# Stebalien/drand

Hardware: AMD Instinct MI355X
Metric: verified beacon rounds/sec, 10M-round chained BLS12-381 chain (higher is better)
Workload: dtype u32 (14x28-bit limb Fp, int32 VALU); 1 GPU; configs[1] shape at the metric's size: chained G2 chain, per-round pairing verify; rounds_total=10000000, rounds_per_gpu=10000000, seg_len=64, scheme=pedersen-bls-chained, mode=per-round, parallelism=shard1

## Files before the change

### __graft_entry__.py

```python
import json
import os
import subprocess
import sys

ROOT = os.path.dirname(os.path.abspath(__file__))
CSRC = os.path.join(ROOT, "drand_amd", "csrc")
LIB = os.path.join(ROOT, "drand_amd", "libdrand_gpu.so")
AB_LIB = os.path.join(ROOT, "drand_amd", "libdrand_gpu_ab.so")
INGEST = os.path.join(ROOT, "drand_amd", "libdrand_ingest.so")
HOSTSIM_SRC = os.path.join(ROOT, "tests", "hostsim", "hostsim.hip")
HOSTSIM = os.path.join(ROOT, "tests", "hostsim", "libdrand_hostsim.so")


def _run(cmd):
    print("+", " ".join(cmd), flush=True)
    subprocess.check_call(cmd, cwd=ROOT)


def build():
    os.environ.setdefault("PYTORCH_ROCM_ARCH", "gfx950")
    hip = ["hipcc", "--offload-arch=gfx950", "-O3", "-std=c++17", "-shared", "-fPIC"]
    ab_cmd = hip + ["-DDG_AB_KNOBS", "-o", AB_LIB, os.path.join(CSRC, "capi.hip")]
    print("+", " ".join(ab_cmd), "&", flush=True)
    ab = subprocess.Popen(ab_cmd, cwd=ROOT)
    try:
        _run(hip + ["-o", LIB, os.path.join(CSRC, "capi.hip")])
    finally:
        if ab.wait() != 0:
            raise subprocess.CalledProcessError(ab.returncode, ab_cmd)
    _run(["g++", "-O3", "-std=c++17", "-fPIC", "-shared", "-Wall", "-o", INGEST, os.path.join(CSRC, "ingest.cpp")])
    _run(["hipcc", "-O2", "-std=c++17", "--cuda-host-only", "-fPIC", "-shared", "-o", HOSTSIM, HOSTSIM_SRC])
    _run(["hipcc", "-O2", "-std=c++17", "--cuda-host-only", "-fPIC", "-shared", "-o",
          os.path.join(ROOT, "tests", "hostsim", "libdrand_reduce_lazy.so"),
          os.path.join(ROOT, "tests", "hostsim", "reduce_lazy.hip")])
    _run(["hipcc", "-O2", "-std=c++17", "--cuda-host-only", "-fPIC", "-shared", "-o",
          os.path.join(ROOT, "tests", "hostsim", "libdrand_miller6.so"),
          os.path.join(ROOT, "tests", "hostsim", "miller6.hip")])
    mk = os.path.join(ROOT, "oracle", "c", "Makefile")
    if os.path.exists(mk):
        _run(["make", "-C", os.path.join(ROOT, "oracle", "c"), "-j8"])
    sys.path.insert(0, ROOT)
    import drand_amd
    from drand_amd import _lib, ingest
    _lib.load()
    assert ingest.load() is not None


def smoke():
    sys.path.insert(0, ROOT)
    import torch
    assert torch.cuda.is_available(), "smoke() needs a GPU"
    from drand_amd.chain import Beacon, Verifier, hash_to_g2
    from drand_amd.scheme import get_scheme_by_id_with_default
    with open(os.path.join(ROOT, "tests", "golden", "chain_chained_s1.json")) as f:
        g = json.load(f)
    v = Verifier(get_scheme_by_id_with_default("pedersen-bls-chained"), device=0)
    beacons = [Beacon(bytes.fromhex(r["prev"]), r["round"], bytes.fromhex(r["sig"])) for r in g["rounds"][:8]]
    beacons += [Beacon(bytes.fromhex(c["prev"]), c["round"], bytes.fromhex(c["sig"])) for c in g["corrupted"]]
    expect = [0] * 8 + [c["reason"] for c in g["corrupted"]]
    got = v.verify_reasons(beacons, bytes.fromhex(g["pk"])).tolist()
    assert got == expect, (got, expect)
    with open(os.path.join(ROOT, "tests", "golden", "hash_to_g2.json")) as f:
        h = json.load(f)["cases"][:4]
    out = hash_to_g2([bytes.fromhex(c["msg"]) for c in h])
    assert [o.hex() for o in out] == [c["h"] for c in h]
    print("smoke ok:", len(beacons), "beacons verified on", torch.cuda.get_device_name(0))


if __name__ == "__main__":
    build()
```

### drand_amd/_lib.py

```python
import ctypes
import sys
import os
import threading

_HERE = os.path.dirname(os.path.abspath(__file__))
LIB_PATH = os.environ.get("DRAND_GPU_LIB") or os.path.join(_HERE, "libdrand_gpu.so")
AB_LIB_PATH = os.path.join(_HERE, "libdrand_gpu_ab.so")
AB_KNOBS = frozenset({"DGPU_DEC_OVERLAP", "DGPU_MSM_SEG", "DGPU_LANE_SLICES", "DGPU_KB_NORM", "DGPU_RLC_DESCENT_STEP",
                      "DGPU_RLC_LOCALIZE", "DGPU_G1_LINES", "DGPU_SUBGROUP", "DGPU_RECOVER", "DGPU_RECOVER_ROWS",
                      "DGPU_KB_INV_CHAIN", "DGPU_KB_TEST_FLAG", "DGPU_TEST_ALLOC_CAP", "DGPU_STAGE",
                      "DGPU_ENG_XW", "DGPU_TEST_STAGE_ONLY", "DGPU_LINES_WAVE", "DGPU_KB_PAIR", "DGPU_TEST_FORCE_EXC",
                      "DGPU_REDUCE_NORM", "DGPU_KEYED_RANGE", "DGPU_TEST_MILLER_MARK"})

DGPU_OK = 0
DGPU_EINVAL = -1
DGPU_EDEVICE = -2
DGPU_ENOMEM = -3
DGPU_EUNSUPPORTED = -4
DGPU_ENOKEY = -5

SCHEME_CHAINED = 0
SCHEME_UNCHAINED = 1
SCHEME_UNCHAINED_G1 = 2
SCHEME_G1_RFC9380 = 3

MODE_PER_ROUND = 0
MODE_RLC = 1

REASON_OK = 0
REASON_DECODE = 1
REASON_SUBGROUP = 2
REASON_PAIRING = 3
REASON_INFINITY = 4
REASON_KEY = 5

_c = ctypes
_P = _c.c_void_p
SYMBOLS = [
    ("dgpu_abi_version", _c.c_int, []),
    ("dgpu_last_error", _c.c_char_p, []),
    ("dgpu_open", _c.c_int, [_c.c_int, _c.POINTER(_P)]),
    ("dgpu_close", None, [_P]),
    ("dgpu_scheme_from_name", _c.c_int, [_c.c_char_p]),
    ("dgpu_set_pubkey", _c.c_int, [_P, _c.c_int, _P, _c.c_size_t]),
    ("dgpu_verify_batch", _c.c_int, [_P, _c.c_int, _c.c_size_t, _P, _P, _c.c_size_t, _P, _P, _c.c_size_t, _P,
                                     _c.c_int, _c.c_uint64, _P, _P]),
    ("dgpu_verify_batch_device", _c.c_int, [_P, _c.c_int, _c.c_size_t, _P, _P, _c.c_size_t, _P, _P, _c.c_size_t,
                                            _P, _c.c_int, _c.c_uint64, _P, _P, _P]),
    ("dgpu_set_profiling", _c.c_int, [_P, _c.c_int]),
    ("dgpu_staging_stats", _c.c_int, [_P, _c.POINTER(_c.c_double), _c.POINTER(_c.c_double), _c.POINTER(_c.c_uint64)]),
    ("dgpu_synchronize", _c.c_int, [_P]),
    ("dgpu_stage_times", _c.c_int, [_P, _c.POINTER(_c.c_float), _c.c_int, _c.POINTER(_c.c_char_p)]),
    ("dgpu_digest_batch", _c.c_int, [_P, _c.c_int, _c.c_size_t, _P, _P, _c.c_size_t, _P, _P]),
    ("dgpu_hash_to_g2", _c.c_int, [_P, _c.c_size_t, _P, _P]),
    ("dgpu_hash_to_g1", _c.c_int, [_P, _c.c_int, _c.c_size_t, _P, _P]),
    ("dgpu_derive_pubkey", _c.c_int, [_P, _c.c_int, _P, _P, _c.c_size_t]),
    ("dgpu_make_chain", _c.c_int, [_P, _c.c_int, _P, _c.c_size_t, _c.c_size_t, _P, _P, _P, _P]),
    ("dgpu_set_group", _c.c_int, [_P, _c.c_int, _c.c_int, _P]),
    ("dgpu_set_group_scheme", _c.c_int, [_P, _c.c_int, _c.c_int, _c.c_int, _P, _c.c_size_t]),
    ("dgpu_recover_batch_device", _c.c_int, [_P, _c.c_size_t, _P, _c.c_size_t, _P, _c.c_size_t, _P, _P, _P, _P, _P]),
    ("dgpu_make_partials", _c.c_int, [_P, _c.c_size_t, _P, _c.c_size_t, _P, _P, _P, _c.c_size_t, _P]),
    ("dgpu_make_partials_scheme", _c.c_int, [_P, _c.c_int, _c.c_size_t, _P, _c.c_size_t, _P, _P, _P, _c.c_size_t,
                                             _P]),
    ("dgpu_recover_batch", _c.c_int, [_P, _c.c_size_t, _P, _c.c_size_t, _P, _c.c_size_t, _P, _P, _P, _P]),
    ("dgpu_shard_range", None, [_c.c_size_t, _c.c_int, _c.c_int, _c.POINTER(_c.c_size_t), _c.POINTER(_c.c_size_t)]),
    ("dgpu_verify_beacons", _c.c_int, [_P, _c.c_int, _P, _c.c_size_t, _c.c_size_t, _P, _P, _c.c_size_t, _P, _P,
                                       _c.c_size_t, _P, _c.c_int, _c.c_uint64, _P, _P]),
    ("dgpu_verify_beacons_device", _c.c_int, [_P, _c.c_int, _P, _c.c_size_t, _c.c_size_t, _P, _P, _c.c_size_t, _P,
                                              _P, _c.c_size_t, _P, _c.c_int, _c.c_uint64, _P, _P, _P]),
    ("dgpu_decode_rows_device", _c.c_int, [_P, _c.c_size_t, _P, _c.c_size_t, _P, _P, _P, _P, _c.c_size_t, _P, _P,
                                           _c.c_size_t, _P, _P, _P]),
    ("dgpu_verify_rows", _c.c_int, [_P, _c.c_int, _P, _c.c_size_t, _c.c_size_t, _P, _P, _P, _c.c_size_t, _c.c_size_t,
                                    _c.c_int, _c.c_uint64, _P, _P, _P, _P]),
    ("dgpu_faulty_rounds_device", _c.c_int, [_P, _c.c_uint64, _c.c_size_t, _c.c_size_t, _P, _P, _P, _P, _P, _P,
                                             _c.c_size_t, _P, _c.c_size_t, _P, _P]),
    ("dgpu_check_rows", _c.c_int, [_P, _c.c_int, _P, _c.c_size_t, _c.c_size_t, _P, _P, _P, _P, _c.c_size_t,
                                   _c.c_size_t, _c.c_int, _c.c_uint64, _c.c_uint64, _c.c_size_t, _P, _P, _c.c_size_t,
                                   _P, _P, _c.c_size_t, _P, _P]),
    ("dgpu_verify_segment", _c.c_int, [_P, _c.c_int, _P, _c.c_size_t, _c.c_uint64, _c.c_size_t, _P, _c.c_size_t, _P,
                                       _P, _c.c_size_t, _c.c_int, _c.c_uint64, _P, _P, _P]),
    ("dgpu_verify_segment_device", _c.c_int, [_P, _c.c_int, _P, _c.c_size_t, _c.c_uint64, _c.c_size_t, _P,
                                              _c.c_size_t, _P, _P, _c.c_size_t, _c.c_int, _c.c_uint64, _P, _P, _P,
                                              _P]),
    ("dgpu_verify_segment_shard_device", _c.c_int, [_P, _c.c_int, _P, _c.c_size_t, _c.c_uint64, _c.c_size_t, _P,
                                                    _c.c_size_t, _P, _P, _P, _c.c_int, _c.c_uint64, _P, _P, _P, _P]),
    ("dgpu_rlc_root_segment_device", _c.c_int, [_P, _c.c_int, _P, _c.c_size_t, _c.c_uint64, _c.c_size_t, _P,
                                                _c.c_size_t, _P, _P, _c.c_size_t, _P, _P, _c.c_uint64, _P, _P]),
    ("dgpu_rlc_root_bytes", _c.c_int, [_c.c_int]),
    ("dgpu_rlc_root_device", _c.c_int, [_P, _c.c_int, _P, _c.c_size_t, _c.c_size_t, _P, _P, _c.c_size_t, _P, _P,
                                        _c.c_size_t, _P, _c.c_uint64, _P, _P]),
    ("dgpu_rlc_finish_device", _c.c_int, [_P, _c.c_size_t, _P, _P, _P, _P]),
    ("dgpu_verify_recovered", _c.c_int, [_P, _c.c_int, _P, _c.c_size_t, _c.c_size_t, _P, _c.c_size_t, _P, _P,
                                         _c.c_size_t, _P, _c.c_int, _c.c_uint64, _P, _P]),
    ("dgpu_hash_to_curve", _c.c_int, [_P, _c.c_int, _c.c_size_t, _P, _c.c_size_t, _P, _P]),
    ("dgpu_sign", _c.c_int, [_P, _c.c_int, _P, _c.c_size_t, _P, _c.c_size_t, _P, _P]),
# ... 148 lines not shown
```

### drand_amd/csrc/capi.hip

```cpp
#include <hip/hip_runtime.h>
#include <dlfcn.h>
#include <rccl/rccl.h>
#include <algorithm>
#include <atomic>
#include <chrono>
#include <condition_variable>
#include <deque>
#include <cstdarg>
#include <cstdio>
#include <cstdlib>
#include <cstring>
#include <mutex>
#include <random>
#include <string>
#include <thread>
#include <vector>

#include "../../include/drand_gpu.h"
#include "copy_pool.h"
#include "kernels.cuh"
#include "pairing_engine.cuh"
#include "miller6_kernels.cuh"
#include "lines_thread.cuh"
#include "kb_thread.cuh"
#include "recover.cuh"
#include "g1sig.cuh"
#include "rlc_msm.cuh"
#include "recover_g1.cuh"
#include "ingest_row.cuh"
#include "check_rows.cuh"
#include "keyed.cuh"
#include "scratch_layouts.h"
#include "record_arrays.h"

using namespace dgpu;

namespace {

thread_local std::string g_last_error;

int set_err(int code, const char* fmt, ...) __attribute__((format(printf, 2, 3)));
int set_err(int code, const char* fmt, ...) {
  char buf[512];
  va_list ap;
  va_start(ap, fmt);
  vsnprintf(buf, sizeof buf, fmt, ap);
  va_end(ap);
  g_last_error = buf;
  return code;
}

#define HIP_TRY(expr)                                                                             \
  do {                                                                                            \
    hipError_t _e = (expr);                                                                       \
    if (_e != hipSuccess) return set_err(DGPU_EDEVICE, "%s: %s", #expr, hipGetErrorString(_e)); \
  } while (0)
#define RC_TRY(expr)                  \
  do {                                \
    if (int _rc = (expr)) return _rc; \
  } while (0)

#ifdef DG_AB_KNOBS
size_t g_test_alloc_cap = 0;
#endif
struct DevBuf {
  void* p = nullptr;
  size_t cap = 0;
  DevBuf() = default;
  DevBuf(const DevBuf&) = delete;
  DevBuf& operator=(const DevBuf&) = delete;
  DevBuf(DevBuf&& o) noexcept : p(o.p), cap(o.cap) { o.p = nullptr, o.cap = 0; }
  DevBuf& operator=(DevBuf&& o) noexcept {
    if (this != &o) {
      release();
      p = o.p, cap = o.cap;
      o.p = nullptr, o.cap = 0;
    }
    return *this;
  }
  ~DevBuf() { release(); }
  int ensure(size_t bytes) {
    if (bytes <= cap) return DGPU_OK;
#ifdef DG_AB_KNOBS
    if (g_test_alloc_cap && bytes > g_test_alloc_cap)
      return set_err(DGPU_ENOMEM, "hipMalloc(%zu): test cap %zu", bytes, g_test_alloc_cap);
#endif
    if (p) {
      (void)hipDeviceSynchronize();
      (void)hipFree(p);
    }
    p = nullptr;
    cap = 0;
    hipError_t e = hipMalloc(&p, bytes ? bytes : 1);
    if (e != hipSuccess) return set_err(DGPU_ENOMEM, "hipMalloc(%zu): %s", bytes, hipGetErrorString(e));
    cap = bytes;
    return DGPU_OK;
  }
  void release() {
    if (p) (void)hipFree(p);
    p = nullptr;
    cap = 0;
  }
  template <class T>
  T* as() const { return static_cast<T*>(p); }
  uint32_t* u32() const { return as<uint32_t>(); }
// ... 39 lines not shown
  z = (z ^ (z >> 30)) * 0xBF58476D1CE4E5B9ull;
  z = (z ^ (z >> 27)) * 0x94D049BB133111EBull;
  return z ^ (z >> 31);
}

inline bool sig_on_g1(int scheme) { return scheme == DGPU_SCHEME_UNCHAINED_G1 || scheme == DGPU_SCHEME_G1_RFC9380; }
inline bool scheme_known(int scheme) { return scheme >= DGPU_SCHEME_CHAINED && scheme <= DGPU_SCHEME_G1_RFC9380; }

constexpr size_t ENG_CHUNK = 1048576;
constexpr size_t ENG_CHUNK_MIN = 16384;
constexpr size_t LANE_MIN = 262144;
constexpr int KEY_SLOTS = 8;
constexpr size_t STAGE_SLOT_BYTES = 16u << 20;
constexpr int STAGE_COPY_THREADS = 8;

struct lane_scratch {
  DevBuf h_pts, sig_pts, h_z, h_pre, h_tmp;
  DevBuf lines, f, n1, kb;
};

struct key_entry {
  bool used = false;
  bool g2key = false;
  uint8_t bytes[96] = {};
  g1_key pk{};
  DevBuf consts, table;
  uint64_t stamp = 0;
};

template <class F>
auto with_src(const msg_src_host& m, F&& f) {
  if (m.linked == SRC_HALO) {
    msg_src_halo h{};
    static_cast<msg_src&>(h) = m;
    h.first_round = m.first_round;
    h.g0 = m.g0;
    h.halo = m.halo;
    h.halo_len = m.halo_len;
    return f(static_cast<const msg_src_halo&>(h));
  }
  return m.linked ? f(static_cast<const msg_src_linked&>(m)) : f(static_cast<const msg_src&>(m));
}
#define SRC_KERNEL(K, src) K<std::decay_t<decltype(src)>>

template <class F>
auto with_group(bool g1, F&& f) {
  return g1 ? f(G1Ops{}) : f(G2Ops{});
}
#define GROUP_OF(gr) std::decay_t<decltype(gr)>

}

struct dgpu_ctx {
  int device = -1;
  hipStream_t stream = nullptr;
  hipStream_t stream2 = nullptr;
  hipEvent_t lane_ev[2] = {nullptr, nullptr};
  hipEvent_t cof_ev[2] = {nullptr, nullptr};
  hipEvent_t done = nullptr;
  std::mutex mu;
  key_entry keys[KEY_SLOTS];
  key_entry* cur = nullptr;
  uint64_t clock = 0;
  DevBuf eng_consts;
  lane_scratch lane[2];
  DevBuf status;
  DevBuf rlc_tree, rlc_idx, rlc_fail, rlc_h, rlc_s, rlc_st, rlc_root;
  DevBuf rlc_conf, rlc_fsum;
  DevBuf msm_aos, msm_flags, msm_counts, msm_list, msm_buckets, msm_runs, msm_root, msm_part;
  bool fe_gs = false;
  size_t fe_gs_max = 16384;
  size_t kb_inv_chain = 16;
  size_t kb_test_flag = 0;
  int lanes = 2;
  size_t lane_slices = 2;
  size_t eng_chunk = ENG_CHUNK;
  size_t chunk_retries = 0;
  bool kb_thread = true;
  bool kb_norm_chain = true;
  bool rlc_localize = true;
  int rlc_descent_step = 3;
  bool lines_thread = true;
  bool miller6 = true;
  size_t thr_min = 65536;
  size_t rlc_min = 131072;
  bool fused_fixed = true;
  bool decode_subgroup = false;
  int grp_t = 0, grp_n = 0;
  int grp_scheme = DGPU_SCHEME_CHAINED;
  bool grp_g1 = false;
  key_entry grp_key;
  DevBuf grp_stage, rec_slots;
  DevBuf grp_commits, grp_table, rec_msgs, rec_parts, rec_plen, rec_hidx, rec_pk, rec_idx, rec_lam, rec_out, rec_ok,
      rec_pts, rec_vpk, rec_sel, rec_part, rec_st;
  DevBuf grp_wtab, rec_cls, rec_x_list, rec_x_msgs, rec_x_parts, rec_x_plen, rec_x_out, rec_x_ok, rec_x_st;
  DevBuf rec_tab, rec_tabz, rec_tabpre;
  DevBuf rec_tab_rows;
  bool recover_exact = false;
  size_t cof_engine_max = 16384;
  DevBuf cof_tmp;
  bool dec_overlap = true;
  bool msm_seg = true;
  int n_cu = 256;
  bool recover_rows = true;
  void* ring[2] = {nullptr, nullptr};
  hipEvent_t ring_ev[2] = {nullptr, nullptr};
  bool ring_busy[2] = {false, false};
  int ring_next = 0;
  hipStream_t stream_copy = nullptr;
  float last_stage_ms = 0.f;
  double last_stage_host_ms = 0.0;
  bool test_stage_only = false;
  size_t last_stage_bytes = 0;
  bool test_miller_mark = false;
  bool kb_pair = false;
  bool reduce_norm = false;
  bool lines_wave = false;
  int eng_xw = 0;
  bool stage_pageable = false;
  DevBuf in_rounds, in_sigs, in_sig_len, in_prev, in_prev_len, in_msgs, in_msg_len, out_bits, out_reason, out_rand, misc;
  DevBuf in_rows, in_row_ok;
  DevBuf in_keys;
  DevBuf chk, chk_out;
  DevBuf in_halo, in_halo_len;
  DevBuf in_key_idx, ky_tab, ky_keys, ky_rlc, ky_exact;
  size_t keyed_range = 0;
  void* ky_host = nullptr;
  size_t ky_host_cap = 0;
  hipEvent_t ky_ev = nullptr;
  bool ky_ev_used = false;
  bool profile = false;
  std::vector<hipEvent_t> ev;
  std::vector<const char*> stage_name;
  int n_ev = 0;
  bool ev_overflow = false;
  bool rlc_pending = false;
  verify_args rlc_args{};
  uint8_t rlc_pk[96] = {};
  size_t rlc_pk_len = 0;
};

namespace {

struct stream_order {
  dgpu_ctx* c;
  hipStream_t s;
  stream_order(dgpu_ctx* c_, hipStream_t s_) : c(c_), s(s_) { (void)hipStreamWaitEvent(s, c->done, 0); }
  ~stream_order() { (void)hipEventRecord(c->done, s); }
};

template <int N>
struct stream_scratch {
  hipStream_t s;
  DevBuf b[N];
  explicit stream_scratch(hipStream_t s_) : s(s_) {}
  ~stream_scratch() { (void)hipStreamSynchronize(s); }
};

struct side_join {
  hipStream_t side, main;
  hipEvent_t ev;
  bool armed;
  side_join(hipStream_t side_, hipStream_t main_, hipEvent_t ev_) : side(side_), main(main_), ev(ev_), armed(side_ != nullptr) {}
  void release() { armed = false; }
  ~side_join() {
    if (armed && hipEventRecord(ev, side) == hipSuccess) (void)hipStreamWaitEvent(main, ev, 0);
  }
};

hipStream_t caller_stream(void* stream) { return (hipStream_t)stream; }

constexpr int STAGE_EVENTS_MAX = 4096;
void mark(dgpu_ctx* c, hipStream_t s, const char* name = nullptr) {
  if (!c->profile) return;
  if (c->n_ev >= STAGE_EVENTS_MAX) {
    c->ev_overflow = true;
    return;
  }
  if ((size_t)c->n_ev == c->ev.size()) {
    hipEvent_t e = nullptr;
    if (hipEventCreate(&e) != hipSuccess) return;
    c->ev.push_back(e);
    c->stage_name.push_back(nullptr);
  }
  (void)hipEventRecord(c->ev[c->n_ev], s);
  c->stage_name[c->n_ev] = name;
  c->n_ev++;
}

void call_reset(dgpu_ctx* c) {
  c->n_ev = 0;
  c->ev_overflow = false;
  c->rlc_pending = false;
}

int upload_eng_consts(DevBuf* dst, const g1_key* key, bool unit_points = false) {
  eng_const_block cb;
// ... 59 lines not shown
  memcpy(gw + 42, gen.y.c1.l, 56);
  hipStream_t s = c->stream;
  hipError_t err = hipMemcpyAsync(d_in, pk, 96, hipMemcpyHostToDevice, s);
  if (err == hipSuccess) err = hipMemcpyAsync(d_g2, gw, sizeof gw, hipMemcpyHostToDevice, s);
  if (err != hipSuccess) return set_err(DGPU_EDEVICE, "set_pubkey: %s", hipGetErrorString(err));
  RC_TRY(launch(k_decode_g2_pk, dim3(1), dim3(64), s, d_in, d_pk, d_rc));
  int drc = -1;
  err = hipMemcpyAsync(&drc, d_rc, sizeof drc, hipMemcpyDeviceToHost, s);
  if (err == hipSuccess) err = hipStreamSynchronize(s);
  if (err != hipSuccess) return set_err(DGPU_EDEVICE, "set_pubkey: %s", hipGetErrorString(err));
  if (drc != DEC_OK) return set_err(DGPU_EINVAL, "public key rejected (decode code %d)", drc);
  RC_TRY(launch(k_eng_lines, dim3(1), dim3(ENG_BLOCK), s, 1, 0, 1, d_pk, 1, nullptr, d_g2, nullptr, unit.u32(),
                e->table.u32(), nullptr, nullptr));
  err = hipStreamSynchronize(s);
  if (err != hipSuccess) return set_err(DGPU_EDEVICE, "set_pubkey lines: %s", hipGetErrorString(err));
  return DGPU_OK;
}

int get_key_locked(dgpu_ctx* c, int scheme, const uint8_t* pk, size_t len, key_entry** out) {
  if (!pk) return set_err(DGPU_EINVAL, "null public key");
  if (!scheme_known(scheme)) return set_err(DGPU_EINVAL, "bad scheme %d", scheme);
  const bool g2key = sig_on_g1(scheme);
  const size_t want = g2key ? 96 : 48;
  if (len != want)
    return set_err(DGPU_EINVAL, "public key must be %zu bytes (compressed %s), got %zu", want, g2key ? "G2" : "G1", len);
  key_entry* victim = nullptr;
  for (key_entry& e : c->keys) {
    if (e.used && e.g2key == g2key && !memcmp(e.bytes, pk, want)) {
      e.stamp = ++c->clock;
      *out = &e;
      return DGPU_OK;
    }
    if (!victim || (!e.used && victim->used) || (e.used == victim->used && e.stamp < victim->stamp)) victim = &e;
  }
  HIP_TRY(hipEventSynchronize(c->done));
  if (c->cur == victim) c->cur = nullptr;
  victim->used = false;
  int rc = g2key ? decode_g2_key_locked(c, victim, pk) : decode_g1_key_locked(c, victim, pk);
  if (rc) return rc;
  victim->used = true;
  victim->g2key = g2key;
  memcpy(victim->bytes, pk, want);
  victim->stamp = ++c->clock;
  *out = victim;
  return DGPU_OK;
}

int eng_fe_kb_locked(dgpu_ctx* c, const uint32_t* consts, size_t cnt, size_t capb, size_t r0, uint32_t* f,
                     const uint32_t* n1inv, const eng_kb_layout& kb, uint8_t* st, hipStream_t s) {
  if (capb % ENG_ROUNDS_PER_BLOCK || cnt > capb) return set_err(DGPU_EINVAL, "karabina FE: bad chunk capacity");
  uint32_t *const xbuf = kb.xbuf, *const pbuf = kb.pbuf, *const pre = kb.pre, *const ebuf = kb.ebuf, *const fb = kb.fb;
  uint8_t* const flags = kb.flags;
  const unsigned blocks = grid_for(cnt, ENG_ROUNDS_PER_BLOCK);
  const size_t inv_threads = std::max<size_t>(1, (cnt + c->kb_inv_chain - 1) / c->kb_inv_chain);
  constexpr int nseg = (int)(sizeof(ENG_PROG_FEK_OFF) / sizeof(ENG_PROG_FEK_OFF[0])) - 1;
  static_assert(nseg == 6, "segment 0 + one per exponentiation by |x|");
  for (int seg = 0; seg < nseg; ++seg) {
    if (seg > 0) {
      mark(c, s, "eng_fe_chain");
      const bool kb_thread = c->kb_thread && cnt >= c->thr_min;
      const bool norm_pre = kb_thread && c->kb_norm_chain;
      if (norm_pre && c->kb_pair)
        RC_TRY(launch_n(k_kb_chain_pair<true>, 2 * cnt, 256, s, cnt, xbuf, ebuf));
#ifdef DG_AB_KNOBS
      else if (kb_thread && c->reduce_norm)
        RC_TRY(launch_n(norm_pre ? k_kb_chain_thr<true, false> : k_kb_chain_thr<false, false>, cnt, 256, s, cnt, xbuf,
                        norm_pre ? ebuf : nullptr));
#endif
      else if (kb_thread)
        RC_TRY(launch_n(norm_pre ? k_kb_chain_thr<true> : k_kb_chain_thr<false>, cnt, 256, s, cnt, xbuf,
                        norm_pre ? ebuf : nullptr));
      else
        RC_TRY(launch(k_eng_kb_chain, dim3(grid_for(cnt, 8)), dim3(64), s, cnt, xbuf));
      mark(c, s, "eng_fe_kbinv");
      RC_TRY(launch_n(norm_pre ? k_eng_kb_norm<true> : k_eng_kb_norm<false>, cnt, 256, s, cnt, r0, xbuf, pbuf, ebuf, flags,
                      st, c->kb_test_flag));
      RC_TRY(launch_n(k_eng_inv, inv_threads, 256, s, cnt, r0, pbuf, pre, st));
      RC_TRY(launch_n(k_eng_kb_dec, (size_t)ENG_KB_NSNAP * cnt, 256, s, cnt, xbuf, pbuf, ebuf, flags));
    }
    mark(c, s, "eng_fe");
    const int so = ENG_PROG_FEK_OFF[seg], sl = ENG_PROG_FEK_OFF[seg + 1] - ENG_PROG_FEK_OFF[seg];
    const bool first = seg == 0, last = seg == nseg - 1;
#ifdef DG_AB_KNOBS
    if (c->eng_xw & 2)
      RC_TRY(launch(first || last ? k_eng_fe_seg_xw<ENG_SLOTS_FE> : k_eng_fe_seg_xw<ENG_FEK_MID_SLOTS>,
                    dim3(grid_for(cnt, ENG_XW_ITEMS)), dim3(ENG_XW_BLOCK), s, so, sl, first, last, cnt, r0, consts, f, n1inv,
                    xbuf, flags, fb, st));
    else
#endif
      RC_TRY(launch(k_eng_fe_seg, dim3(blocks), dim3(ENG_BLOCK), s, so, sl, first, last, cnt, r0, consts, f, n1inv, xbuf,
                    flags, fb, st));
  }
  return launch(k_eng_fe_fb, dim3(ENG_FB_GRID), dim3(ENG_BLOCK), s, cnt, r0, consts, f, n1inv, st, flags, fb);
}

struct pairing_job {
  const uint32_t* consts = nullptr;
  size_t n = 0;
  const uint32_t* h = nullptr;
  const uint32_t* sg = nullptr;
  uint8_t* st = nullptr;
  size_t h_stride = 0;
  const uint32_t* h_idx = nullptr;
  const uint32_t* pk_items = nullptr;
  const uint32_t* fixed_table = nullptr;
  lane_scratch* lane = nullptr;
  bool sig_subgroup = false;
  const uint32_t* g1form_keys = nullptr;
};

int eng_pairing_locked(dgpu_ctx* c, const pairing_job& job, hipStream_t s) {
  const uint32_t* const consts = job.consts;
  const size_t n = job.n;
  const uint32_t *const h = job.h, *const sg = job.sg;
  uint8_t* const st = job.st;
  const size_t h_stride = job.h_stride ? job.h_stride : n;
  const uint32_t *const h_idx = job.h_idx, *const pk_items = job.pk_items, *const fixed_table = job.fixed_table;
  lane_scratch& L = job.lane ? *job.lane : c->lane[0];
  const bool sig_subgroup = job.sig_subgroup;
  const uint32_t* const g1form_keys = job.g1form_keys;
  const bool need_lines = !(fixed_table && c->fused_fixed);
  const bool fe_gs = c->fe_gs || n <= c->fe_gs_max;
  int rc;
  size_t cap = 0, cap_blk = 0;
  eng_kb_layout kb{};
  bool retried = false;
  for (;;) {
    const size_t nchunks = (n + c->eng_chunk - 1) / c->eng_chunk;
    cap = (n + nchunks - 1) / nchunks;
    cap = std::min(n, (cap + ENG_ROUNDS_PER_BLOCK - 1) / ENG_ROUNDS_PER_BLOCK * ENG_ROUNDS_PER_BLOCK);
    cap_blk = eng_blocks(cap);
    rc = fe_gs ? DGPU_OK : carve(L.kb, &kb, cap_blk);
    if (!rc && need_lines) rc = L.lines.ensure(eng_blk_words(cap_blk, ENG_LINE_STEPS) * 4);
    if (!rc) rc = L.f.ensure(eng_blk_words(cap_blk, ENG_F_PLANES) * 4);
    if (!rc) rc = L.n1.ensure(eng_n1_words(cap) * 4);
    if (rc != DGPU_ENOMEM || c->eng_chunk <= ENG_CHUNK_MIN || cap <= ENG_CHUNK_MIN) break;
    HIP_TRY(hipStreamSynchronize(s));
    HIP_TRY(hipStreamSynchronize(c->stream));
    HIP_TRY(hipStreamSynchronize(c->stream2));
    for (DevBuf* b : {&L.kb, &L.lines, &L.f, &L.n1}) b->release();
    c->eng_chunk = std::max(ENG_CHUNK_MIN, c->eng_chunk / 2);
    ++c->chunk_retries;
    retried = true;
  }
  if (rc) return rc;
  if (retried) g_last_error.clear();
  uint32_t* lines = need_lines ? L.lines.u32() : nullptr;
  uint32_t* f = L.f.u32();
  uint32_t* n1 = L.n1.u32();
  uint32_t* pre = need_lines ? lines : nullptr;
  if (!pre) {
    if ((rc = c->lane[0].lines.ensure(eng_n1_words(cap) * 4))) return rc;
    pre = c->lane[0].lines.u32();
  }
  uint8_t* const sub_st = sig_subgroup ? st : nullptr;
  for (size_t r0 = 0; r0 < n; r0 += cap) {
    const size_t cnt = std::min(cap, n - r0);
    const dim3 blocks(grid_for(cnt, ENG_ROUNDS_PER_BLOCK)), eng(ENG_BLOCK);
    if (!need_lines) {
      mark(c, s, "eng_miller");
      RC_TRY(launch(k_eng_miller_fixed, blocks, eng, s, n, r0, cnt, consts, h, sg, fixed_table, f, n1));
    } else {
      const bool thr = c->lines_thread && cnt >= c->thr_min;
      if (g1form_keys) {
        mark(c, s, "eng_lines");
        RC_TRY(launch_n(k_lines_thr_g1, 2 * cnt, 256, s, n, r0, cnt, h, h_stride, h_idx, sg, g1form_keys, lines));
      } else if (fixed_table) {
        mark(c, s, "eng_lines_fixed");
        RC_TRY(launch(k_eng_lines_fixed, dim3(blocks.x, ENG_LINE_STEPS), eng, s, n, r0, cnt, h, sg, fixed_table, lines));
      } else if (thr && !pk_items && c->lines_wave) {
        mark(c, s, "eng_lines");
        RC_TRY(launch_n(k_lines_thr<true>, 2 * ((cnt + 63) / 64 * 64), 256, s, n, r0, cnt, h, h_stride, h_idx, sg, pk_items,
                        consts, lines, sub_st));
      } else if (thr) {
// ... 1085 lines not shown
  hipStream_t s = c->stream;
  stream_order ord(c, s);
  if (a.n && (rc = verify_status_host_locked(c, key, a, s))) return rc;
  if (a.n) mark(c, s);
  if ((rc = check_lists_locked(c, first, count, a.n, a.m.rows->d_keys, faulty_cap, left_cap, out, s))) return rc;
  if (reason && a.n) {
    HIP_TRY(hipMemcpyAsync(reason, c->status.p, a.n, hipMemcpyDeviceToHost, s));
    HIP_TRY(hipStreamSynchronize(s));
  }
  return DGPU_OK;
}

void check_lists_store(const check_lists& L, uint64_t* faulty_pos, uint64_t* faulty_val, size_t faulty_cap,
                       uint64_t* n_faulty, uint64_t* left_rows, size_t left_cap, uint64_t* n_left) {
  const size_t nf = std::min(L.pos.size(), faulty_cap), nl = std::min(L.left.size(), left_cap);
  if (nf) memcpy(faulty_pos, L.pos.data(), nf * 8), memcpy(faulty_val, L.val.data(), nf * 8);
  if (nl) memcpy(left_rows, L.left.data(), nl * 8);
  *n_faulty = L.n_faulty;
  *n_left = L.n_left;
}

size_t size_engine_chunk(int lanes) {
  size_t free_b = 0, total_b = 0;
  if (hipMemGetInfo(&free_b, &total_b) != hipSuccess) return ENG_CHUNK;
  const size_t fit = free_b / 2 / ((size_t)std::max(lanes, 1) * eng_bytes_per_round());
  return std::max(ENG_CHUNK_MIN, std::min(ENG_CHUNK, fit));
}

}

extern "C" {

int dgpu_abi_version(void) { return DGPU_ABI_VERSION; }
const char* dgpu_last_error(void) { return g_last_error.c_str(); }

int dgpu_scheme_from_name(const char* name) {
  if (!name) return set_err(DGPU_EINVAL, "null scheme name");
  if (name[0] == 0 || !strcmp(name, "pedersen-bls-chained")) return DGPU_SCHEME_CHAINED;
  if (!strcmp(name, "pedersen-bls-unchained")) return DGPU_SCHEME_UNCHAINED;
  if (!strcmp(name, "bls-unchained-on-g1")) return DGPU_SCHEME_UNCHAINED_G1;
  if (!strcmp(name, "bls-unchained-g1-rfc9380")) return DGPU_SCHEME_G1_RFC9380;
  return set_err(DGPU_EINVAL, "scheme [%s] is not valid", name);
}

void dgpu_shard_range(size_t n, int ndev, int k, size_t* lo, size_t* hi) {
  if (ndev < 1) ndev = 1;
  size_t per = (n + (size_t)ndev - 1) / (size_t)ndev;
  per = (per + 7) & ~(size_t)7;
  size_t a = std::min(n, (size_t)k * per), b = std::min(n, a + per);
  if (k < 0) a = b = 0;
  if (lo) *lo = a;
  if (hi) *hi = b;
}

int dgpu_open(int device, dgpu_ctx** out) {
  if (!out) return set_err(DGPU_EINVAL, "null out");
  *out = nullptr;
  int count = 0;
  hipError_t e = hipGetDeviceCount(&count);
  if (e != hipSuccess || count == 0) return set_err(DGPU_EDEVICE, "no HIP device available (%s)", hipGetErrorString(e));
  if (device < 0 || device >= count) return set_err(DGPU_EINVAL, "device %d out of range (%d devices)", device, count);
  hipDeviceProp_t prop;
  HIP_TRY(hipGetDeviceProperties(&prop, device));
  if (strncmp(prop.gcnArchName, "gfx950", 6) != 0)
    return set_err(DGPU_EDEVICE, "device %d is %s; this library is built for gfx950 only", device, prop.gcnArchName);
  HIP_TRY(hipSetDevice(device));
  dgpu_ctx* c = new dgpu_ctx();
  c->device = device;
  c->n_cu = prop.multiProcessorCount > 0 ? prop.multiProcessorCount : 256;
  const char* fgv = getenv("DGPU_FE_GS_MAX");
  if (fgv && atol(fgv) >= 0) c->fe_gs_max = (size_t)atol(fgv);
  const char* cev = getenv("DGPU_COF_ENGINE_MAX");
  if (cev && atol(cev) >= 0) c->cof_engine_max = (size_t)atol(cev);
  const char* lv = getenv("DGPU_LANES");
  if (lv && !strcmp(lv, "1")) c->lanes = 1;
  const char* ec = getenv("DGPU_ENG_CHUNK");
  c->eng_chunk = (ec && atol(ec) >= 4096) ? (size_t)atol(ec) : size_engine_chunk(c->lanes);
  const char* kcv = getenv("DGPU_KB_CHAIN");
  if (kcv && !strcmp(kcv, "lanes")) c->kb_thread = false;
  const char* lnv = getenv("DGPU_LINES");
  if (lnv && !strcmp(lnv, "engine")) c->lines_thread = false;
  const char* mlv = getenv("DGPU_MILLER");
  if (mlv && !strcmp(mlv, "lanes12")) c->miller6 = false;
  const char* tmv = getenv("DGPU_THR_MIN");
  if (tmv && atol(tmv) >= 0) c->thr_min = (size_t)atol(tmv);
  const char* rmv = getenv("DGPU_RLC_MIN");
  if (rmv && atol(rmv) >= 0) c->rlc_min = (size_t)atol(rmv);
  const char* fev = getenv("DGPU_FE");
  if (fev && !strcmp(fev, "gs")) c->fe_gs = true;
#ifdef DG_AB_KNOBS
  const char* dov = getenv("DGPU_DEC_OVERLAP");
  if (dov && !strcmp(dov, "0")) c->dec_overlap = false;
  const char* msv = getenv("DGPU_MSM_SEG");
  if (msv && !strcmp(msv, "0")) c->msm_seg = false;
  const char* lsv = getenv("DGPU_LANE_SLICES");
  if (lsv && atol(lsv) >= 2 && atol(lsv) <= 64) c->lane_slices = (size_t)atol(lsv);
  const char* knv = getenv("DGPU_KB_NORM");
  if (knv) c->kb_norm_chain = strcmp(knv, "planes") != 0;
  const char* rds = getenv("DGPU_RLC_DESCENT_STEP");
  if (rds && atoi(rds) >= 1 && atoi(rds) <= 8) c->rlc_descent_step = atoi(rds);
  const char* rlv = getenv("DGPU_RLC_LOCALIZE");
  if (rlv && !strcmp(rlv, "0")) c->rlc_localize = false;
  const char* gl = getenv("DGPU_G1_LINES");
  if (gl && !strcmp(gl, "buffer")) c->fused_fixed = false;
  const char* sgv = getenv("DGPU_SUBGROUP");
  if (sgv && !strcmp(sgv, "decode")) c->decode_subgroup = true;
  const char* rcv = getenv("DGPU_RECOVER");
  if (rcv && !strcmp(rcv, "exact")) c->recover_exact = true;
  const char* rrv = getenv("DGPU_RECOVER_ROWS");
  if (rrv && !strcmp(rrv, "0")) c->recover_rows = false;
  const char* kic = getenv("DGPU_KB_INV_CHAIN");
  if (kic && atol(kic) >= 1) c->kb_inv_chain = (size_t)atol(kic);
  const char* ktf = getenv("DGPU_KB_TEST_FLAG");
  if (ktf && atol(ktf) >= 1) c->kb_test_flag = (size_t)atol(ktf);
  const char* mmv = getenv("DGPU_TEST_MILLER_MARK");
  if (mmv) c->test_miller_mark = !strcmp(mmv, "1");
  const char* kpv = getenv("DGPU_KB_PAIR");
  if (kpv) c->kb_pair = !strcmp(kpv, "1");
  const char* rnv = getenv("DGPU_REDUCE_NORM");
  if (rnv) c->reduce_norm = !strcmp(rnv, "1");
  const char* lwv = getenv("DGPU_LINES_WAVE");
  if (lwv) c->lines_wave = !strcmp(lwv, "1");
  const char* xwv = getenv("DGPU_ENG_XW");
  if (xwv) c->eng_xw = atoi(xwv) & 3;
  const char* stv = getenv("DGPU_STAGE");
  if (stv && !strcmp(stv, "pageable")) c->stage_pageable = true;
  const char* krv = getenv("DGPU_KEYED_RANGE");
  if (krv && atol(krv) >= 1) c->keyed_range = (size_t)atol(krv);
  const char* tso = getenv("DGPU_TEST_STAGE_ONLY");
  if (tso && !strcmp(tso, "1")) c->test_stage_only = true;
  const char* tac = getenv("DGPU_TEST_ALLOC_CAP");
  g_test_alloc_cap = tac && atol(tac) >= 0 ? (size_t)atol(tac) : 0;
  {
    const char* fev2 = getenv("DGPU_TEST_FORCE_EXC");
    const int force = fev2 && !strcmp(fev2, "1") ? 1 : 0;
    const hipError_t fe = hipMemcpyToSymbol(HIP_SYMBOL(g_dg_force_exc), &force, sizeof(force));
    if (fe != hipSuccess) {
      delete c;
      return set_err(DGPU_EDEVICE, "DGPU_TEST_FORCE_EXC: %s", hipGetErrorString(fe));
    }
  }
#endif
  e = hipStreamCreateWithFlags(&c->stream, hipStreamNonBlocking);
  if (e == hipSuccess) e = hipStreamCreateWithFlags(&c->stream2, hipStreamNonBlocking);
  if (e == hipSuccess) e = hipEventCreateWithFlags(&c->lane_ev[0], hipEventDisableTiming);
  if (e == hipSuccess) e = hipEventCreateWithFlags(&c->lane_ev[1], hipEventDisableTiming);
  if (e == hipSuccess) e = hipEventCreateWithFlags(&c->cof_ev[0], hipEventDisableTiming);
  if (e == hipSuccess) e = hipEventCreateWithFlags(&c->cof_ev[1], hipEventDisableTiming);
  if (e == hipSuccess) e = hipEventCreateWithFlags(&c->done, hipEventDisableTiming);
  if (e != hipSuccess) {
    dgpu_close(c);
    return set_err(DGPU_EDEVICE, "hipStreamCreate: %s", hipGetErrorString(e));
  }
  if (upload_eng_consts(&c->eng_consts, nullptr) != DGPU_OK) {
    std::string msg = g_last_error;
    dgpu_close(c);
    return set_err(DGPU_EDEVICE, "%s", msg.c_str());
  }
  g_last_error.clear();
  *out = c;
  return DGPU_OK;
}

void dgpu_close(dgpu_ctx* c) {
  if (!c) return;
  (void)hipSetDevice(c->device);
  if (c->stream) (void)hipStreamSynchronize(c->stream);
  if (c->stream2) (void)hipStreamSynchronize(c->stream2);
  if (c->done) (void)hipEventSynchronize(c->done);
  for (hipEvent_t e : c->ev) (void)hipEventDestroy(e);
  for (hipEvent_t e : c->lane_ev)
    if (e) (void)hipEventDestroy(e);
  for (hipEvent_t e : c->cof_ev)
    if (e) (void)hipEventDestroy(e);
  if (c->done) (void)hipEventDestroy(c->done);
  if (c->ky_ev) (void)hipEventDestroy(c->ky_ev);
  if (c->ky_host) (void)hipHostFree(c->ky_host);
  if (c->stream_copy) {
    (void)hipStreamSynchronize(c->stream_copy);
    (void)hipStreamDestroy(c->stream_copy);
  }
  for (int k = 0; k < 2; ++k) {
    if (c->ring_ev[k]) (void)hipEventDestroy(c->ring_ev[k]);
    if (c->ring[k]) (void)hipHostFree(c->ring[k]);
  }
  if (c->stream2) (void)hipStreamDestroy(c->stream2);
  if (c->stream) (void)hipStreamDestroy(c->stream);
  delete c;
}

int dgpu_set_pubkey(dgpu_ctx* c, int scheme, const uint8_t* pk, size_t len) {
  if (!c || !pk) return set_err(DGPU_EINVAL, "null argument");
  std::lock_guard<std::mutex> lk(c->mu);
  HIP_TRY(hipSetDevice(c->device));
  key_entry* k = nullptr;
  int rc = get_key_locked(c, scheme, pk, len, &k);
  if (rc) return rc;
  c->cur = k;
  return DGPU_OK;
// ... 624 lines not shown
```

Before: 2.609 million rounds/s.

## Add six-lane final-exponentiation segment kernel reusing miller6 Fp12 layout

Adds a new kernel for the hard-part final-exponentiation segments (after segment 0). Each item is spread across six lanes that share Fp12 coefficients through LDS, reusing the miller6 multiply and square helpers. When the batch is at least the threshold size, this path replaces the 12-lane k_eng_fe_seg kernel. The goal is better lane utilisation and fewer registers per lane, at the cost of more LDS traffic and hand-written Frobenius and conjugation transforms that must match the old program exactly.

Result: faster. 2.652 million rounds/s, median of 6 (+1.6%).

```diff
diff --git a/__graft_entry__.py b/__graft_entry__.py
--- a/__graft_entry__.py
+++ b/__graft_entry__.py
@@ -36,6 +36,9 @@
     _run(["hipcc", "-O2", "-std=c++17", "--cuda-host-only", "-fPIC", "-shared", "-o",
           os.path.join(ROOT, "tests", "hostsim", "libdrand_miller6.so"),
           os.path.join(ROOT, "tests", "hostsim", "miller6.hip")])
+    _run(["hipcc", "-O2", "-std=c++17", "--cuda-host-only", "-fPIC", "-shared", "-o",
+          os.path.join(ROOT, "tests", "hostsim", "libdrand_feseg6.so"),
+          os.path.join(ROOT, "tests", "hostsim", "feseg6.hip")])
     mk = os.path.join(ROOT, "oracle", "c", "Makefile")
     if os.path.exists(mk):
         _run(["make", "-C", os.path.join(ROOT, "oracle", "c"), "-j8"])
diff --git a/drand_amd/_lib.py b/drand_amd/_lib.py
--- a/drand_amd/_lib.py
+++ b/drand_amd/_lib.py
@@ -10,7 +10,8 @@
                       "DGPU_RLC_LOCALIZE", "DGPU_G1_LINES", "DGPU_SUBGROUP", "DGPU_RECOVER", "DGPU_RECOVER_ROWS",
                       "DGPU_KB_INV_CHAIN", "DGPU_KB_TEST_FLAG", "DGPU_TEST_ALLOC_CAP", "DGPU_STAGE",
                       "DGPU_ENG_XW", "DGPU_TEST_STAGE_ONLY", "DGPU_LINES_WAVE", "DGPU_KB_PAIR", "DGPU_TEST_FORCE_EXC",
-                      "DGPU_REDUCE_NORM", "DGPU_KEYED_RANGE", "DGPU_TEST_MILLER_MARK"})
+                      "DGPU_REDUCE_NORM", "DGPU_KEYED_RANGE", "DGPU_TEST_MILLER_MARK",
+                      "DGPU_TEST_FE_MARK"})
 
 DGPU_OK = 0
 DGPU_EINVAL = -1
diff --git a/drand_amd/csrc/capi.hip b/drand_amd/csrc/capi.hip
--- a/drand_amd/csrc/capi.hip
+++ b/drand_amd/csrc/capi.hip
@@ -21,6 +21,7 @@
 #include "kernels.cuh"
 #include "pairing_engine.cuh"
 #include "miller6_kernels.cuh"
+#include "feseg6_kernels.cuh"
 #include "lines_thread.cuh"
 #include "kb_thread.cuh"
 #include "recover.cuh"
@@ -226,6 +227,7 @@
   int rlc_descent_step = 3;
   bool lines_thread = true;
   bool miller6 = true;
+  bool feseg6 = true;
   size_t thr_min = 65536;
   size_t rlc_min = 131072;
   bool fused_fixed = true;
@@ -257,6 +259,7 @@
   bool test_stage_only = false;
   size_t last_stage_bytes = 0;
   bool test_miller_mark = false;
+  bool test_fe_mark = false;
   bool kb_pair = false;
   bool reduce_norm = false;
   bool lines_wave = false;
@@ -482,14 +485,23 @@
     const int so = ENG_PROG_FEK_OFF[seg], sl = ENG_PROG_FEK_OFF[seg + 1] - ENG_PROG_FEK_OFF[seg];
     const bool first = seg == 0, last = seg == nseg - 1;
 #ifdef DG_AB_KNOBS
-    if (c->eng_xw & 2)
+    if (c->eng_xw & 2) {
       RC_TRY(launch(first || last ? k_eng_fe_seg_xw<ENG_SLOTS_FE> : k_eng_fe_seg_xw<ENG_FEK_MID_SLOTS>,
                     dim3(grid_for(cnt, ENG_XW_ITEMS)), dim3(ENG_XW_BLOCK), s, so, sl, first, last, cnt, r0, consts, f, n1inv,
                     xbuf, flags, fb, st));
-    else
+      continue;
+    }
 #endif
+    if (!first && c->feseg6 && cnt >= c->thr_min) {
+#ifdef DG_AB_KNOBS
+      if (c->test_fe_mark) mark(c, s, "eng_fe_seg6");
+#endif
+      RC_TRY(launch(k_eng_fe_seg6, dim3(grid_for(cnt, M6_ITEMS_PER_WAVE)), dim3(ENG_BLOCK), s, seg, cnt, r0, consts, xbuf,
+                    flags, fb, st));
+    } else {
       RC_TRY(launch(k_eng_fe_seg, dim3(blocks), dim3(ENG_BLOCK), s, so, sl, first, last, cnt, r0, consts, f, n1inv, xbuf,
                     flags, fb, st));
+    }
   }
   return launch(k_eng_fe_fb, dim3(ENG_FB_GRID), dim3(ENG_BLOCK), s, cnt, r0, consts, f, n1inv, st, flags, fb);
 }
@@ -1741,6 +1753,8 @@
   if (lnv && !strcmp(lnv, "engine")) c->lines_thread = false;
   const char* mlv = getenv("DGPU_MILLER");
   if (mlv && !strcmp(mlv, "lanes12")) c->miller6 = false;
+  const char* fsv = getenv("DGPU_FESEG");
+  if (fsv && !strcmp(fsv, "lanes12")) c->feseg6 = false;
   const char* tmv = getenv("DGPU_THR_MIN");
   if (tmv && atol(tmv) >= 0) c->thr_min = (size_t)atol(tmv);
   const char* rmv = getenv("DGPU_RLC_MIN");
@@ -1774,6 +1788,8 @@
   if (ktf && atol(ktf) >= 1) c->kb_test_flag = (size_t)atol(ktf);
   const char* mmv = getenv("DGPU_TEST_MILLER_MARK");
   if (mmv) c->test_miller_mark = !strcmp(mmv, "1");
+  const char* fmv = getenv("DGPU_TEST_FE_MARK");
+  if (fmv) c->test_fe_mark = !strcmp(fmv, "1");
   const char* kpv = getenv("DGPU_KB_PAIR");
   if (kpv) c->kb_pair = !strcmp(kpv, "1");
   const char* rnv = getenv("DGPU_REDUCE_NORM");
diff --git a/drand_amd/csrc/feseg6.cuh b/drand_amd/csrc/feseg6.cuh
--- /dev/null
+++ b/drand_amd/csrc/feseg6.cuh
@@ -0,0 +1,115 @@
+#pragma once
+#include "miller6.cuh"
+
+namespace dgpu {
+
+constexpr int FS6_A = 24;
+static_assert(FS6_A + 2 * M6_LANES == M6_SLOTS, "R takes 6 x 4 slots, A 6 x 2");
+
+enum { FS6_X_NONE = 0, FS6_X_CONJ = 1, FS6_X_FROB1 = 2, FS6_X_FROB2 = 3, FS6_X_SQR = 4 };
+struct fs6_step {
+  int plane, xf;
+  bool conj_r, st_m, st_t2;
+};
+constexpr int FS6_LAST_SEG = (int)(sizeof(ENG_PROG_FEK_OFF) / sizeof(ENG_PROG_FEK_OFF[0])) - 2;
+static_assert(FS6_LAST_SEG == 5, "segment 0, then one per exponentiation by |x|");
+DG_FN int fs6_nsteps(int seg) { return seg == 4 ? 5 : seg == FS6_LAST_SEG ? 9 : 6; }
+DG_FN fs6_step fs6_plan(int seg, int s) {
+  fs6_step p{0, FS6_X_NONE, false, false, false};
+  if (s < ENG_KB_NSNAP - 1) {
+    p.plane = ENG_KB_PL_X0 + 1 + s;
+    p.conj_r = s == ENG_KB_NSNAP - 2;
+    p.st_m = p.conj_r && seg == 4;
+    return p;
+  }
+  const int q = s - (ENG_KB_NSNAP - 1);
+  if (seg == 1 || seg == 2) {
+    p.plane = ENG_KB_PL_M, p.xf = FS6_X_CONJ, p.st_m = true;
+  } else if (seg == 3) {
+    p.plane = ENG_KB_PL_M, p.xf = FS6_X_FROB1, p.st_m = p.st_t2 = true;
+  } else {
+    p.plane = q < 2 ? ENG_KB_PL_T2 : ENG_KB_PL_T;
+    p.xf = q == 0 ? FS6_X_FROB2 : q == 1 ? FS6_X_CONJ : q == 2 ? FS6_X_NONE : FS6_X_SQR;
+  }
+  return p;
+}
+
+DG_FN size_t fs6_plane_off(const m6_lane& L, int plane) { return eng_blk_off(L.blk, ENG_KB_PLANES, plane, L.g, 2 * L.m); }
+DG_FN size_t fs6_item(const m6_lane& L) { return L.blk * ENG_ROUNDS_PER_BLOCK + L.g; }
+
+DG_FN fp2 fs6_ld_plane(const uint32_t* p) {
+  fp2 v;
+#pragma unroll
+  for (int l = 0; l < FP_LIMBS; ++l) {
+    const uint2 w = *reinterpret_cast<const uint2*>(p + l * ENG_WAVE_WORDS);
+    v.c0.l[l] = w.x, v.c1.l[l] = w.y;
+  }
+  return v;
+}
+DG_FN void fs6_st_plane(uint32_t* p, const fp& re, const fp& im) {
+  const fp a = eng_reduce(re), b = eng_reduce(im);
+#pragma unroll
+  for (int l = 0; l < FP_LIMBS; ++l) *reinterpret_cast<uint2*>(p + l * ENG_WAVE_WORDS) = make_uint2(a.l[l], b.l[l]);
+}
+
+DG_FN fp2 fs6_get_a(const uint32_t* it, int m) {
+  const uint32_t* p = it + (FS6_A + 2 * m) * ENG_SLOT_WORDS;
+  return fp2{eng_ld(p), eng_ld(p + ENG_SLOT_WORDS)};
+}
+DG_FN void fs6_put_a(uint32_t* it, int m, const fp2& a) {
+  uint32_t* p = it + (FS6_A + 2 * m) * ENG_SLOT_WORDS;
+  eng_st(p, a.c0);
+  eng_st(p + ENG_SLOT_WORDS, a.c1);
+}
+
+DG_FN fp fs6_neg(const fp& x) { return eng_reduce(eng_cyc_sum(fp_zero(), x, true)); }
+
+DG_FN fp fs6_const(const uint32_t* consts, int slot) {
+  fp a;
+#pragma unroll
+  for (int l = 0; l < FP_LIMBS; ++l) a.l[l] = consts[(slot - ENG_C_ONE) * ENG_SLOT_WORDS + l];
+  return a;
+}
+
+template <bool CONJ>
+DG_FN fp2 fs6_mul_const(const fp2& x, const fp& g0, const fp& g1) {
+  const fp nx1 = fp_sub_lz(fp_zero(), x.c1);
+  uint64_t col[2 * FP_LIMBS];
+  col[2 * FP_LIMBS - 1] = 0;
+  fp2 r;
+  m6_mac<true>(col, g0, x.c0);
+  m6_mac<false>(col, g1, CONJ ? x.c1 : nx1);
+  r.c0 = fp_redc_cols(col);
+  m6_mac<true>(col, g1, x.c0);
+  m6_mac<false>(col, g0, CONJ ? nx1 : x.c1);
+  r.c1 = fp_redc_cols(col);
+  return r;
+}
+
+DG_FN fp2 fs6_xform(const fp2& a, int xf, int m, const uint32_t* consts) {
+  if (xf == FS6_X_CONJ) return (m & 1) ? fp2{fs6_neg(a.c0), fs6_neg(a.c1)} : a;
+  if (xf == FS6_X_FROB1) {
+    const fp g0 = fs6_const(consts, m ? ENG_C_G1 + 2 * (m - 1) : ENG_C_ONE);
+    const fp g1 = m ? fs6_const(consts, ENG_C_G1 + 2 * (m - 1) + 1) : fp_zero();
+    return fs6_mul_const<true>(a, g0, g1);
+  }
+  if (xf == FS6_X_FROB2) return fs6_mul_const<false>(a, fs6_const(consts, m ? ENG_C_G2 + (m - 1) : ENG_C_ONE), fp_zero());
+  return a;
+}
+
+DG_FN void fs6_mul(const uint32_t* it, int m, fp& re, fp& im) {
+  m6_term tm[M6_LANES];
+#pragma unroll
+  for (int i = 0; i < M6_LANES; ++i) {
+    const bool wrap = i > m;
+    tm[i].a = it + i * M6_COEF_WORDS + (wrap ? 2 * ENG_SLOT_WORDS : 0);
+    tm[i].b = it + (FS6_A + 2 * (m - i + (wrap ? M6_LANES : 0))) * ENG_SLOT_WORDS;
+    tm[i].sh = 0;
+  }
+  m6_fp2_sum<M6_LANES, false>(tm, nullptr, re, im);
+}
+
+DG_FN bool fs6_eq(const fp& x, const fp& K) { return fp_is_zero(eng_reduce(fp_norm(fp_sub_lz(x, K)))); }
+DG_FN bool fs6_is_one(const fp& re, const fp& im, int m) { return fs6_eq(re, m == 0 ? fp_one() : fp_zero()) && fs6_eq(im, fp_zero()); }
+
+}
diff --git a/drand_amd/csrc/feseg6_kernels.cuh b/drand_amd/csrc/feseg6_kernels.cuh
--- /dev/null
+++ b/drand_amd/csrc/feseg6_kernels.cuh
@@ -0,0 +1,64 @@
+#pragma once
+#include "feseg6.cuh"
+#include "pairing_engine.cuh"
+
+namespace dgpu {
+
+__global__ void __launch_bounds__(ENG_BLOCK, 2) k_eng_fe_seg6(int seg, size_t cnt, size_t r0,
+                                                           const uint32_t* __restrict__ consts,
+                                                           uint32_t* __restrict__ xbuf,
+                                                           const uint8_t* __restrict__ flags, uint32_t* __restrict__ fb,
+                                                           uint8_t* __restrict__ status) {
+  __shared__ uint32_t lds[M6_ITEMS_PER_WAVE * M6_ITEM_WORDS];
+  const int lane = threadIdx.x & 63;
+  const m6_lane L = m6_lane_id(cnt, blockIdx.x, lane);
+  const int m = L.m;
+  uint32_t* it = lds + L.gi * M6_ITEM_WORDS;
+  fp re, im;
+  {
+    const fp2 x = fs6_ld_plane(xbuf + fs6_plane_off(L, ENG_KB_PL_X0));
+    re = x.c0, im = x.c1;
+  }
+  m6_store(it, m, re, im);
+  asm volatile("" ::: "memory");
+  const int ns = fs6_nsteps(seg);
+#pragma unroll 1
+  for (int s = 0; s < ns; ++s) {
+    const fs6_step p = fs6_plan(seg, s);
+    if (p.xf == FS6_X_SQR) {
+      const fp2 t = fs6_get_a(it, m);
+      m6_store(it, m, t.c0, t.c1);
+      asm volatile("" ::: "memory");
+      fp2 sq;
+      m6_sqr(it, m, sq.c0, sq.c1);
+      asm volatile("" ::: "memory");
+      fs6_put_a(it, m, sq);
+      m6_store(it, m, re, im);
+    } else {
+      fs6_put_a(it, m, fs6_xform(fs6_ld_plane(xbuf + fs6_plane_off(L, p.plane)), p.xf, m, consts));
+    }
+    asm volatile("" ::: "memory");
+    fs6_mul(it, m, re, im);
+    asm volatile("" ::: "memory");
+    if (p.conj_r && (m & 1)) re = fs6_neg(re), im = fs6_neg(im);
+    m6_store(it, m, re, im);
+    asm volatile("" ::: "memory");
+    if (L.valid) {
+      if (p.st_m) fs6_st_plane(xbuf + fs6_plane_off(L, ENG_KB_PL_M), re, im);
+      if (p.st_t2) fs6_st_plane(xbuf + fs6_plane_off(L, ENG_KB_PL_T2), re, im);
+    }
+  }
+  if (seg == FS6_LAST_SEG) {
+    const uint64_t vote = __ballot(fs6_is_one(re, im, m));
+    const bool all = ((vote >> (M6_LANES * L.gi)) & 0x3Full) == 0x3Full;
+    const size_t i = fs6_item(L);
+    const bool flagged = L.valid && flags[i];
+    if (L.valid && m == 0 && !all && !flagged && status[r0 + i] == ST_OK) status[r0 + i] = ST_PAIRING;
+    const uint64_t fl = __ballot(flagged);
+    constexpr int HALF = ENG_ROUNDS_PER_BLOCK * M6_LANES;
+    if (lane == 0 && (fl & ((1ull << HALF) - 1)) != 0) fb[1 + atomicAdd(fb, 1u)] = (uint32_t)L.blk;
+    if (lane == HALF && (fl >> HALF) != 0) fb[1 + atomicAdd(fb, 1u)] = (uint32_t)L.blk;
+  }
+}
+
+}
```
